# aaletov/open-pcc-metric

Hardware: AMD Instinct MI355X
Metric: Mpoints/s for symmetric D1+D2 PSNR, N_ref=N_deg=1M (higher is better)
Workload: dtype f64

## Files before the change

open_pcc_metric_amd/csrc/pccm_brick.hip:

```cpp
#include "pccm_brick.h"

namespace pccm {

#define BRICK_STAMP(k)                                                                       \
    do {                                                                                     \
        if (STAMP) {                                                                         \
            const unsigned long long now_ = __builtin_amdgcn_s_memtime();                    \
            t_sum[k] += now_ - t_last;         \
            t_last = now_;                                                                   \
        }                                                                                    \
    } while (0)

__device__ __forceinline__ void load_normal(const NNOut &o, int row, double &a, double &b, double &c)
{
    if (o.nrm32) {
        const float4 t = o.nrm32[row];
        a = (double)t.x; b = (double)t.y; c = (double)t.z;
    } else {
        const double *np = o.nrm + 3 * (int64_t)row;
        a = np[0]; b = np[1]; c = np[2];
    }
}

template <bool SELF, int BY, int BZ, bool STAMP, int ABL, bool N32, int PL>
// ... 299 lines not shown
        }
        BRICK_STAMP(5);
        const float thr = __builtin_fmaf(best, 1.0f + 0x1.0p-18f, 2.0e-36f);
        bool settled = false;
        if (ABL & 4) {
            if (best < 0.0f) store_result(out, qrow, 0.0, 0.0, 0);
            settled = true;
        } else if (bestpos != 0xffffffffu && best < 1.0e30f && second > thr) {
            uint32_t f = (bestpos - 8u - lds0) >> 2;
            float partner;
            {
                const v2f px = *reinterpret_cast<const v2f *>(s_x + f), py = *reinterpret_cast<const v2f *>(s_y + f),
                          pz = *reinterpret_cast<const v2f *>(s_z + f);
                const v2f dx = qxx - px, dy = qyy - py, dz = qzz - pz;
                v2f dd = dx * dx;
                dd = __builtin_elementwise_fma(dy, dy, dd);
                dd = __builtin_elementwise_fma(dz, dz, dd);
                float d0 = dd.x, d1 = dd.y;
                if (SELF) {
                    d0 = (__float_as_int(s_r[f]) == qrow) ? kBigF : d0;
                    d1 = (__float_as_int(s_r[f + 1]) == qrow) ? kBigF : d1;
                }
                const bool first = d0 == best;
                partner = first ? d1 : d0;
                f += first ? 0u : 1u;
            }
            float L = face32(q.x, cx, dimx, bp.h32[0], bp.face_lo[0], bp.face_hi[0]);
            L = fminf(L, face32(q.y, cy, dimy, bp.h32[1], bp.face_lo[1], bp.face_hi[1]));
            L = fminf(L, face32(q.z, cz, dimz, bp.h32[2], bp.face_lo[2], bp.face_hi[2]));
            settled = partner > thr && L > 0.0f && best * 1.00001f < L * L * 0.99999f;
            const float wx = s_x[f], wy = s_y[f], wz = s_z[f];
            const int wrow = __float_as_int(s_r[f]);
            if (settled && defer) {
                store_result_rec(out, qrow, wx, wy, wz, wrow);
            } else if (settled) {
                const double rx = (double)wx, ry = (double)wy, rz = (double)wz;
                const double d64 = gdist64(qx, qy, qz, rx, ry, rz);
                double p = 0.0;
                if (fuse) {
                    double e0 = N32 ? (double)nraw.x : n0, e1 = N32 ? (double)nraw.y : n1, e2 = N32 ? (double)nraw.z : n2;
                    if (!fuse_row) {
                        load_normal(out, wrow, e0, e1, e2);
                    }
                    const double ex = __dsub_rn(qx, rx), ey = __dsub_rn(qy, ry), ez = __dsub_rn(qz, rz);
                    p = __dmul_rn(ex, e0);
                    p = __fma_rn(ey, e1, p);
                    p = __fma_rn(ez, e2, p);
                }
                store_result(out, qrow, d64, p, wrow);
            }
        }
        if (!settled) {
            const uint32_t pos = atomicAdd(&J.counters[1], 1u);
            reinterpret_cast<float4 *>(J.tail)[pos] = q;
        }
        if (hn) {
            rn = query_row(qnext);
            qn = load_query(qnext, rn);
            gather_row_normal(__float_as_int(qn.w), fuse_row);
        }
        qi = qnext;
        have = hn;
        if (STAMP) {
            BRICK_STAMP(q_iter == 0 ? 3 : 4);
            ++q_iter;
        }
    }
// ... 189 lines not shown
```

open_pcc_metric_amd/csrc/pccm_color.hip:

```cpp
#include "pccm_internal.h"

namespace pccm {

__constant__ double kColourMatrix[2][9] = {
    {0.2126, 0.7152, 0.0722, -0.1146, -0.3854, 0.5, 0.5, -0.4542, -0.0458},
    {0.25, 0.5, 0.25, 1, 0, -1, -0.5, 1, -0.5},
};

__device__ __forceinline__ void to_scheme(int scheme, const double c[3], double o[3])
{
    if (scheme == 0) {
        o[0] = c[0]; o[1] = c[1]; o[2] = c[2];
        return;
    }
    const double *m = kColourMatrix[scheme - 1];
#pragma unroll
    for (int r = 0; r < 3; ++r) o[r] = fma(m[3 * r + 2], c[2], fma(m[3 * r], c[0], m[3 * r + 1] * c[1]));
}

__device__ __forceinline__ unsigned long long max_key(double v)
{
    return isnan(v) ? 0x7ff8000000000000ull : (unsigned long long)__double_as_longlong(v);
}

struct ByteLut {
    double v[256];
    constexpr ByteLut() : v() {
        for (int k = 0; k < 256; ++k) v[k] = (double)k / 255.0;
    }
};
__constant__ ByteLut c_byte_lut = ByteLut();

template <bool U8>
__global__ __launch_bounds__(256) void k_color_rows(const double *__restrict__ own, const double *__restrict__ other,
                                                    const uint32_t *__restrict__ own8, const uint32_t *__restrict__ other8,
                                                    const int32_t *__restrict__ rows, const float4 *__restrict__ recs, int64_t n, int64_t n_other,
                                                    int scheme, double scale, int what, double *__restrict__ out,
                                                    unsigned long long *__restrict__ maxkeys, unsigned int *__restrict__ bad,
                                                    const double *__restrict__ other_q)
{
    __shared__ unsigned long long s_max[4][3];
    __shared__ double s_lut[U8 ? 256 : 1];
    if (U8) {
        s_lut[threadIdx.x] = c_byte_lut.v[threadIdx.x];
        __syncthreads();
    }
    const int64_t i = (int64_t)blockIdx.x * 256 + threadIdx.x;
    unsigned long long key[3] = {0ull, 0ull, 0ull};
    if (i < n) {
        double a[3], b[3], ta[3], tb[3];
        int64_t r = rows ? rows[i] : (int64_t)__float_as_int(recs[i].w);
        if (r < 0 || r >= n_other) {
            atomicOr(bad, 1u);
            r = 0;
        }
        if (U8) {
            const uint32_t pa = own8[i];
            a[0] = s_lut[pa & 255u]; a[1] = s_lut[(pa >> 8) & 255u]; a[2] = s_lut[(pa >> 16) & 255u];
        } else {
            a[0] = own[3 * i]; a[1] = own[3 * i + 1]; a[2] = own[3 * i + 2];
        }
        if (other_q) {
            b[0] = other_q[3 * i]; b[1] = other_q[3 * i + 1]; b[2] = other_q[3 * i + 2];
        } else if (U8) {
            const uint32_t pb = other8[r];
            b[0] = s_lut[pb & 255u]; b[1] = s_lut[(pb >> 8) & 255u]; b[2] = s_lut[(pb >> 16) & 255u];
        } else {
            b[0] = other[3 * r]; b[1] = other[3 * r + 1]; b[2] = other[3 * r + 2];
        }
        to_scheme(scheme, a, ta);
        to_scheme(scheme, b, tb);
#pragma unroll
        for (int c = 0; c < 3; ++c) {
            const double diff = scale * (ta[c] - tb[c]);
            const double sq = diff * diff;
            if (what == 4) {
                out[(int64_t)c * n + i] = sq;
                key[c] = max_key(sq);
            } else {
                out[3 * i + c] = what == 0 ? ta[c] : what == 1 ? tb[c] : what == 2 ? diff : sq;
            }
        }
    }
    if (what != 4 || !maxkeys) return;
// ... 623 lines not shown
```

open_pcc_metric_amd/csrc/pccm_grid.h:

```cpp
#pragma once
#include "pccm_internal.h"

namespace pccm {

struct GridGeom {
    int dim[3];
    int morton = 0;
    double org[3], h[3], inv_h[3], slack[3];
};

__device__ __forceinline__ uint32_t spread3(uint32_t v)
{
    v &= 0x3ffu;
    v = (v | (v << 16)) & 0x030000ffu;
    v = (v | (v << 8)) & 0x0300f00fu;
    v = (v | (v << 4)) & 0x030c30c3u;
    v = (v | (v << 2)) & 0x09249249u;
    return v;
}

__device__ __forceinline__ int cell_coord(double v, double org, double inv_h, int dim)
{
    double t = floor(__dmul_rn(__dsub_rn(v, org), inv_h));
    t = t < 0.0 ? 0.0 : t;
// ... 64 lines not shown
    *reinterpret_cast<float4 *>(&recs[p]) = r;
}

struct BuildJob {
    const double *x64;
    const float *x32;
    int64_t row0, n;
    uint32_t *cs;
    uint32_t *occ = nullptr;
    const Rec32 *sp = nullptr;
};

struct BuildJobs {
    BuildJob j[2];
    int njobs;
    int64_t total;
};

int sort_by_cell(pccm_ctx *ctx, const BuildJobs &jobs, const GridGeom &g, int64_t ncells, void *recs, bool rec32,
                 uint32_t *zero = nullptr, int nzero = 0);

int64_t scan_tiles(int64_t m);

struct NNOut {
    double *rec;
    int stride;
    const double *nrm;
    const float4 *nrm32;
    int64_t row_base;
    int normal_mode;
    int layout;
};

__device__ __forceinline__ void store_result_rec(const NNOut &o, int qrow, float rx, float ry, float rz, int wrow)
{
    reinterpret_cast<float4 *>(o.rec)[qrow - o.row_base] = make_float4(rx, ry, rz, __int_as_float(wrow));
}

__device__ __forceinline__ void store_result(const NNOut &o, int qrow, double d2, double p, int wrow)
{
    double *dst = o.rec + (int64_t)(qrow - o.row_base) * o.stride;
    *reinterpret_cast<double2 *>(dst) = make_double2(d2, p);
    if (o.stride == 4) *reinterpret_cast<double2 *>(dst + 2) = make_double2(__longlong_as_double((long long)(uint32_t)wrow), 0.0);
}

__device__ __forceinline__ void emit_result(const NNOut &o, int qrow, double qx, double qy, double qz, int wrow, double d2,
                                            double rx, double ry, double rz)
{
    if (o.layout == 1) {
        const bool has = wrow >= 0;
        store_result_rec(o, qrow, (float)(has ? rx : qx), (float)(has ? ry : qy), (float)(has ? rz : qz), wrow);
        return;
    }
    double p = 0.0;
    if (o.nrm && wrow >= 0) {
        const int64_t k = (o.normal_mode == PCCM_NORMAL_ROW) ? (int64_t)qrow : (int64_t)wrow;
        const double ex = __dsub_rn(qx, rx), ey = __dsub_rn(qy, ry), ez = __dsub_rn(qz, rz);
        p = __dmul_rn(ex, o.nrm[3 * k]);
        p = __fma_rn(ey, o.nrm[3 * k + 1], p);
        p = __fma_rn(ez, o.nrm[3 * k + 2], p);
    }
    store_result(o, qrow, d2, p, wrow);
}


__device__ __forceinline__ void emit_result_lookup(const NNOut &o, const double *__restrict__ s64, int qrow, double qx, double qy,
                                                   double qz, int wrow, double d2)
{
    double rx = 0.0, ry = 0.0, rz = 0.0;
    if ((o.nrm || o.layout == 1) && wrow >= 0) {
        rx = s64[3 * (int64_t)wrow];
        ry = s64[3 * (int64_t)wrow + 1];
        rz = s64[3 * (int64_t)wrow + 2];
    }
    emit_result(o, qrow, qx, qy, qz, wrow, d2, rx, ry, rz);
}

struct QueryJob {
    const void *qrecs;
    const void *qbase;
    const uint32_t *qcs;
    int64_t nq, nchunks;
    const uint32_t *cs;
    const uint32_t *occ;
// ... 68 lines not shown
```

open_pcc_metric_amd/csrc/pccm_internal.h:

```cpp
#pragma once
#include <hip/hip_runtime.h>
#include <stdint.h>
#include <mutex>
#include <string>
#include <vector>

#include "pccm.h"
#include "pccm_slot.h"

#ifdef PCCM_DIAG
#define PCCM_DIAG_ENV(name) getenv(name)
#else
#define PCCM_DIAG_ENV(name) (static_cast<const char *>(nullptr))
#endif

namespace pccm {

constexpr int kScanThreads = 256;
constexpr int kScanTile = 1024;
constexpr int kTileVec = kScanTile / 4 * 3;
constexpr int kGranule = 64;
constexpr float kBig32 = 3.0e38f;
constexpr float kPadCoord = 1.0e18f;
constexpr double kMaxAbsCoord = 1.0e15;


struct Cloud {
    int64_t n = 0;
    int64_t n_pad = 0;
    float4 *xyz32 = nullptr;
    double *xyz64 = nullptr;
    float4 *xyz32r = nullptr;
    size_t cap32r = 0;
    double *nrm64 = nullptr;
    float4 *nrm32 = nullptr;
    bool nrm_exact32 = false;
    int64_t n_nrm = 0;
    const void *nrm_host = nullptr;
    int nrm_host_dtype = 0;
    bool nrm_deferred = false;
// ... 570 lines not shown
```

open_pcc_metric_amd/csrc/pccm_point.hip:

```cpp
#include "pccm_internal.h"
#include "pccm_reduce_shape.h"

namespace pccm {

__device__ __forceinline__ unsigned long long order_key(double v)
{
    unsigned long long b = (unsigned long long)__double_as_longlong(v);
    return (b >> 63) ? ~b : (b | 0x8000000000000000ull);
}

template <typename T>
__global__ __launch_bounds__(256) void k_ingest_points(const T *__restrict__ src, int64_t n, int64_t n_pad,
                                                       float *__restrict__ x32, double *__restrict__ x64, float4 *__restrict__ x32r,
                                                       unsigned long long *__restrict__ stats)
{
    __shared__ unsigned long long s_mx[4], s_lo[4][3], s_hi[4][3];
    __shared__ int s_cnt[4][3];
    unsigned long long mx = 0;
    unsigned long long lo[3] = {~0ull, ~0ull, ~0ull}, hi[3] = {0ull, 0ull, 0ull};
    int inexact = 0, bad = 0, frac = 0;
    for (int64_t i = (int64_t)blockIdx.x * 256 + threadIdx.x; i < n_pad; i += (int64_t)gridDim.x * 256) {
        if (i < n) {
            double v[3];
            float f[3];
#pragma unroll
            for (int a = 0; a < 3; ++a) {
                v[a] = (double)src[3 * i + a];
                f[a] = (float)v[a];
                inexact += ((double)f[a] != v[a]) ? 1 : 0;
                frac += (floor(v[a]) != v[a]) ? 1 : 0;
                bad += isfinite(v[a]) ? 0 : 1;
                unsigned long long b = (unsigned long long)__double_as_longlong(fabs(v[a]));
                mx = b > mx ? b : mx;
                x64[3 * i + a] = v[a];
// ... 73 lines not shown
}

int launch_ingest_points(pccm_ctx *ctx, const void *src, int dtype, int64_t n, int64_t n_pad, float4 *x32,
                         double *x64, float4 *x32r, unsigned long long *stats)
{
    ProfScope ps(ctx, PCCM_K_INGEST);
    const int64_t blocks = (n_pad + 255) / 256;
    dim3 grid((unsigned)(blocks < 256 ? blocks : 256));
    if (dtype == PCCM_F32)
        PCCM_LAUNCH(ctx, (k_ingest_points<float>), grid, dim3(256), 0, ctx->stream, (const float *)src, n, n_pad, (float *)x32, x64, x32r, stats);
    else
        PCCM_LAUNCH(ctx, (k_ingest_points<double>), grid, dim3(256), 0, ctx->stream, (const double *)src, n, n_pad, (float *)x32, x64, x32r, stats);
    PCCM_HIP(hipGetLastError());
    return PCCM_OK;
}

int launch_ingest_normals(pccm_ctx *ctx, const void *src, int dtype, int64_t n, double *out, float *out32, unsigned long long *stats)
{
    ProfScope ps(ctx, PCCM_K_INGEST);
    const int64_t n3 = 3 * n;
    dim3 grid((unsigned)((n3 + 255) / 256));
    if (dtype == PCCM_F32)
        PCCM_LAUNCH(ctx, (k_ingest_normals<float>), grid, dim3(256), 0, ctx->stream, (const float *)src, n3, out, out32, stats);
    else
        PCCM_LAUNCH(ctx, (k_ingest_normals<double>), grid, dim3(256), 0, ctx->stream, (const double *)src, n3, out, out32, stats);
    PCCM_HIP(hipGetLastError());
    return PCCM_OK;
}

__device__ __forceinline__ void point_row(const PointJob &J, int64_t i)
{
    const int64_t gi = J.q_begin + i;
    if (J.metric == PCCM_METRIC_ANGULAR) {
        const int64_t j = J.recs ? (int64_t)__float_as_int(J.recs[i].w) : (int64_t)J.idx[i];
        J.val[i] = angular_similarity(J.inrm + 3 * gi, J.nrm + 3 * j);
        return;
    }
    if (is_ssim_metric(J.metric)) {
        const int64_t j = J.recs ? (int64_t)__float_as_int(J.recs[i].w) : (int64_t)J.idx[i];
        J.val[i] = ssim_similarity(J.inrm[gi], J.nrm[j]);
        return;
    }
    const int64_t j = J.idx[i];
    const double *r = J.c64 ? J.c64 + 3 * i : J.r64 + 3 * j;
    const double ex = __dsub_rn(J.q64[3 * gi], r[0]);
    const double ey = __dsub_rn(J.q64[3 * gi + 1], r[1]);
    const double ez = __dsub_rn(J.q64[3 * gi + 2], r[2]);
    if (J.metric == PCCM_METRIC_D1) {
        J.val[3 * i] = ex;
        J.val[3 * i + 1] = ey;
        J.val[3 * i + 2] = ez;
        return;
    }
    const double *nv = (J.normal_mode == PCCM_NORMAL_ROW) ? J.nrm + 3 * gi : J.cn64 ? J.cn64 + 3 * i : J.nrm + 3 * j;
    double p = __dmul_rn(ex, nv[0]);
    p = __fma_rn(ey, nv[1], p);
    p = __fma_rn(ez, nv[2], p);
    J.val[i] = (J.metric == PCCM_METRIC_PROJ) ? p : __dmul_rn(p, p);
}

__global__ __launch_bounds__(256) void k_point_jobs(PointJobs jobs)
{
    const int64_t i0 = (int64_t)blockIdx.x * 256 + threadIdx.x;
    if (i0 >= jobs.off[jobs.njobs]) return;
    int jb = 0;
#pragma unroll
    for (int k = 1; k < 4; ++k)
        if (k < jobs.njobs && i0 >= jobs.off[k]) jb = k;
    point_row(jobs.j[jb], i0 - jobs.off[jb]);
}

int launch_point_jobs(pccm_ctx *ctx, const PointJobs &jobs)
{
    const int64_t total = jobs.off[jobs.njobs];
    if (total <= 0) return PCCM_OK;
    ProfScope ps(ctx, PCCM_K_POINT);
    PCCM_LAUNCH(ctx, k_point_jobs, dim3((unsigned)((total + 255) / 256)), dim3(256), 0, ctx->stream, jobs);
    PCCM_HIP(hipGetLastError());
    return PCCM_OK;
}

struct UnitView {
    const double *val;
    int stride, off0, off1, sq0, sq1;
    int defer;
    int64_t nrm_rows;
    const double *nrm64;
    const float4 *nrm32;
    const float4 *q32;
    int64_t row0;
};

__device__ __forceinline__ void matched_fields(const float4 rec, const float4 *__restrict__ q32, int defer, const double *__restrict__ nrm64,
                                               const float4 *__restrict__ nrm32, int64_t row, bool want_proj, double &d2, double &proj,
                                               int64_t nrm_rows = 0)
{
    const float4 q = q32[row];
    const double qx = (double)q.x, qy = (double)q.y, qz = (double)q.z;
    const double ex = __dsub_rn(qx, (double)rec.x), ey = __dsub_rn(qy, (double)rec.y), ez = __dsub_rn(qz, (double)rec.z);
    d2 = __dadd_rn(__dadd_rn(__dmul_rn(ex, ex), __dmul_rn(ey, ey)), __dmul_rn(ez, ez));
    proj = 0.0;
    if (want_proj && defer != 3) {
        double n0, n1, n2;
        int64_t nr = row;
        if (defer >= 4) {
            nr = (int64_t)__float_as_int(rec.w);
            nr = nr < 0 ? 0 : (nr >= nrm_rows ? nrm_rows - 1 : nr);
        }
        if (defer == 1 || defer == 4) {
            const float4 t = nrm32[nr];
            n0 = (double)t.x; n1 = (double)t.y; n2 = (double)t.z;
        } else {
            n0 = nrm64[3 * nr]; n1 = nrm64[3 * nr + 1]; n2 = nrm64[3 * nr + 2];
        }
        proj = __dmul_rn(ex, n0);
        proj = __fma_rn(ey, n1, proj);
        proj = __fma_rn(ez, n2, proj);
    }
}

__device__ __forceinline__ UnitView unit_view(const UnitJob &J)
{
    UnitView w;
    w.val = J.val;
    w.stride = J.stride;
    w.off0 = J.c[0].off; w.off1 = J.c[1].off;
    w.sq0 = J.c[0].square; w.sq1 = J.c[1].square;
    w.defer = J.defer; w.nrm64 = J.nrm64; w.nrm32 = J.nrm32; w.q32 = J.q32; w.row0 = J.row0; w.nrm_rows = J.nrm_rows;
    return w;
}

__device__ __forceinline__ void unit_load(const UnitView &J, int64_t i, double v[2])
{
    if (J.stride >= 2 && J.defer) {
        matched_fields(reinterpret_cast<const float4 *>(J.val)[i], J.q32, J.defer, J.nrm64, J.nrm32, J.row0 + i, true, v[0], v[1], J.nrm_rows);
    } else if (J.stride >= 2) {
        const double2 t = *reinterpret_cast<const double2 *>(&J.val[i * J.stride]);
        v[0] = t.x;
        v[1] = t.y;
    } else {
        v[0] = v[1] = J.val[i];
    }
}

__device__ __forceinline__ void unit_pick(const UnitView &J, double v[2])
{
    if (J.stride >= 2) {
        const double x = v[0], y = v[1];
        v[0] = J.off0 ? y : x;
        v[1] = J.off1 ? y : x;
// ... 133 lines not shown
#pragma unroll
    for (int r = 0; r < kSelPerCol; ++r) {
        if (!own[r]) continue;
        uint32_t *g = S.hist + ((size_t)p * kSelMax + s0 + r) * kSelBins;
        for (int b = t; b < kSelBins; b += 256) {
            const uint32_t c = lh[r * kSelBins + b];
            if (c) atomicAdd(&g[b], c);
        }
    }
}

__device__ __forceinline__ double dmin_raw(double a, double b)
{
    double r;
    asm("v_min_f64 %0, %1, %2" : "=v"(r) : "v"(a), "v"(b));
    return r;
}
__device__ __forceinline__ double dmax_raw(double a, double b)
{
    double r;
    asm("v_max_f64 %0, %1, %2" : "=v"(r) : "v"(a), "v"(b));
    return r;
}

struct UnitCols {
    static constexpr int NC = 2;
    const UnitView V;
    const int ncols;
    __device__ __forceinline__ explicit UnitCols(const UnitJob &J) : V(unit_view(J)), ncols(J.ncols) {}
    __device__ __forceinline__ bool live(int c) const { return c < ncols; }
    static __device__ __forceinline__ double min(double a, double b) { return fmin(a, b); }
    static __device__ __forceinline__ double max(double a, double b) { return fmax(a, b); }
    __device__ __forceinline__ void one(int64_t i, double v[2]) const { unit_load(V, i, v); unit_pick(V, v); }
    __device__ __forceinline__ void leaf(int64_t base, int k, double v[kLeaf / 8][2]) const
    {
        __builtin_assume((base & (kLeaf - 1)) == 0 && k >= 0 && k < 8);
        if (V.stride >= 2 && V.defer) {
#pragma unroll
            for (int j = 0; j < kLeaf / 8; ++j) unit_load(V, base + 8 * j + k, v[j]);
        } else if (V.stride >= 2) {
#pragma unroll
            for (int j = 0; j < kLeaf / 8; ++j) {
                const double2 t = *reinterpret_cast<const double2 *>(&V.val[(base + 8 * j + k) * V.stride]);
                v[j][0] = t.x;
                v[j][1] = t.y;
            }
        } else {
#pragma unroll
            for (int j = 0; j < kLeaf / 8; ++j) v[j][0] = v[j][1] = V.val[base + 8 * j + k];
        }
#pragma unroll
        for (int j = 0; j < kLeaf / 8; ++j) unit_pick(V, v[j]);
    }
};

template <int STRIDE, int CFG, int DEFER>
struct LeanCols {
    static constexpr int NC = CFG == 0 ? 2 : 1;
    const double *__restrict__ val, *__restrict__ nrm64;
    const float4 *__restrict__ nrm32, *__restrict__ q32;
    const int64_t row0, nrm_rows;
    __device__ __forceinline__ explicit LeanCols(const UnitJob &J)
        : val(J.val), nrm64(J.nrm64), nrm32(J.nrm32), q32(J.q32), row0(J.row0), nrm_rows(J.nrm_rows) {}
    __device__ __forceinline__ bool live(int) const { return true; }
    static __device__ __forceinline__ double min(double a, double b) { return dmin_raw(a, b); }
    static __device__ __forceinline__ double max(double a, double b) { return dmax_raw(a, b); }
    __device__ __forceinline__ void one(int64_t i, double out[NC]) const { at(val + i * STRIDE, i, out); }
    __device__ __forceinline__ void at(const double *p, int64_t i, double out[NC]) const
    {
        double x, y = 0.0;
        if (DEFER) {
            matched_fields(*reinterpret_cast<const float4 *>(p), q32, DEFER, nrm64, nrm32, row0 + i, CFG != 1, x, y, nrm_rows);
        } else if (STRIDE >= 2) {
            const double2 q = *reinterpret_cast<const double2 *>(p);
            x = q.x; y = q.y;
        } else {
            x = *p;
        }
        if (CFG == 0) { out[0] = x; out[1] = __dmul_rn(y, y); }
        else out[0] = CFG == 1 ? x : __dmul_rn(y, y);
    }
    __device__ __forceinline__ void leaf(int64_t base, int k, double v[kLeaf / 8][NC]) const
    {
        __builtin_assume((base & (kLeaf - 1)) == 0 && k >= 0 && k < 8);
        const int64_t first = base + k;
        const double *p = val + first * STRIDE;
#pragma unroll
        for (int j = 0; j < kLeaf / 8; ++j) at(p + (int64_t)j * 8 * STRIDE, first + 8 * j, v[j]);
    }
};

__device__ __forceinline__ int unit_job_at(const int64_t (&off)[9], int njobs, int64_t pos)
{
    int jb = 0;
#pragma unroll
    for (int k = 1; k < 8; ++k)
        if (k < njobs && pos >= off[k]) jb = k;
    return jb;
}

template <class P>
__device__ __forceinline__ void unit_leaves(const UnitJobs &jobs, int jb, int64_t t)
{
    constexpr int NC = P::NC;
    __shared__ double ls[NC][32], lmn[NC][32], lmx[NC][32];
    const UnitJob &J = jobs.j[jb];
    const P cols(J);
    const int64_t ns = J.ns, nunits = J.nunits;
    const int64_t lane = t - jobs.uoff[jb], u = lane >> 3;
    const int k = threadIdx.x & 7, grp = threadIdx.x >> 3;
    const int64_t base = u * kLeaf;
    const bool live = u < nunits;
    const int64_t cnt = !live ? 0 : ((ns - base < kLeaf) ? ns - base : kLeaf);
    double r[NC], mn[NC], mx[NC];
    if (cnt == kLeaf) {
        double v[kLeaf / 8][NC];
        cols.leaf(base, k, v);
#pragma unroll
        for (int c = 0; c < NC; ++c) {
            r[c] = v[0][c];
            mn[c] = mx[c] = v[0][c];
#pragma unroll
            for (int j = 1; j < kLeaf / 8; ++j) {
                r[c] = __dadd_rn(r[c], v[j][c]);
                mn[c] = P::min(mn[c], v[j][c]);
                mx[c] = P::max(mx[c], v[j][c]);
            }
        }
    } else {
#pragma unroll
        for (int c = 0; c < NC; ++c) { r[c] = 0.0; mn[c] = INFINITY; mx[c] = -INFINITY; }
        for (int64_t e = k; e < cnt; e += 8) {
            double w[NC];
            cols.one(base + e, w);
#pragma unroll
            for (int c = 0; c < NC; ++c) {
                r[c] = __dadd_rn(r[c], w[c]);
                mn[c] = P::min(mn[c], w[c]);
                mx[c] = P::max(mx[c], w[c]);
            }
        }
    }
#pragma unroll
    for (int c = 0; c < NC; ++c) {
#pragma unroll
        for (int off = 1; off < 8; off <<= 1) {
            r[c] = __dadd_rn(r[c], __shfl_xor(r[c], off));
            mn[c] = P::min(mn[c], __shfl_xor(mn[c], off));
            mx[c] = P::max(mx[c], __shfl_xor(mx[c], off));
        }
    }
    if (k == 0) {
#pragma unroll
        for (int c = 0; c < NC; ++c) {
            double *ou = cols.live(c) ? J.c[c].out_units : nullptr;
            if (live && ou) {
                ou[u] = r[c];
                ou[nunits + u] = mn[c];
                ou[2 * nunits + u] = mx[c];
            }
            ls[c][grp] = r[c];
// ... 21 lines not shown
    }
}

template <class P>
__device__ __forceinline__ void unit_tail(const UnitJobs &jobs, int64_t c0)
{
    if (c0 >= jobs.toff[jobs.njobs]) return;
    const int jb = unit_job_at(jobs.toff, jobs.njobs, c0);
    const UnitJob &J = jobs.j[jb];
    const P cols(J);
    const int64_t e = c0 - jobs.toff[jb];
    double v[P::NC];
    cols.one(J.tail_first + e, v);
#pragma unroll
    for (int c = 0; c < P::NC; ++c)
        if (cols.live(c)) J.c[c].out_tail[e] = v[c];
}

__global__ __launch_bounds__(256) void k_unit_jobs(UnitJobs jobs)
{
    __shared__ __attribute__((aligned(16))) unsigned char sel_smem[kSelLds];
    if (jobs.sel.pass) {
        unit_select(jobs, sel_smem);
        return;
    }
    const int64_t t = (int64_t)blockIdx.x * 256 + threadIdx.x;
    const int64_t unit_threads = jobs.uoff[jobs.njobs];
    if (t < unit_threads)
        unit_leaves<UnitCols>(jobs, __builtin_amdgcn_readfirstlane(unit_job_at(jobs.uoff, jobs.njobs, t)), t);
    else
        unit_tail<UnitCols>(jobs, t - unit_threads);
}

template <int STRIDE, int CFG, int DEFER = 0>
__global__ __launch_bounds__(256) void k_unit_lean(UnitJobs jobs)
{
    const int64_t t = (int64_t)blockIdx.x * 256 + threadIdx.x;
    const int64_t unit_threads = jobs.uoff[jobs.njobs];
    if ((int64_t)blockIdx.x * 256 < unit_threads)
        unit_leaves<LeanCols<STRIDE, CFG, DEFER>>(jobs, unit_job_at(jobs.uoff, jobs.njobs, (int64_t)blockIdx.x * 256), t);
    else
        unit_tail<LeanCols<STRIDE, CFG, DEFER>>(jobs, t - unit_threads);
}

__global__ __launch_bounds__(64) void k_publish(unsigned long long *done)
{
    if (threadIdx.x == 0) {
        __builtin_amdgcn_fence(__ATOMIC_RELEASE, "");
        asm volatile("s_waitcnt vmcnt(0)" ::: "memory");
        __hip_atomic_fetch_add(done, 1ull, __ATOMIC_RELAXED, __HIP_MEMORY_SCOPE_SYSTEM);
    }
}

struct LeanKernel {
    ReduceShape shape;
    void (*stub)(UnitJobs);
};
template <int STRIDE, int CFG, int DEFER>
constexpr LeanKernel lean() { return {{STRIDE, CFG, DEFER}, k_unit_lean<STRIDE, CFG, DEFER>}; }
static constexpr LeanKernel kLeanKernels[] = {
    lean<1, 1, 0>(),
    lean<2, 0, 0>(),
    lean<2, 1, 0>(),
    lean<2, 2, 0>(),
    lean<4, 0, 0>(),
    lean<4, 1, 0>(),
    lean<4, 2, 0>(),
    lean<2, 0, 1>(),
// ... 79 lines not shown
int launch_unit_select(pccm_ctx *ctx, UnitJobs &jobs)
{
    UnitSelect &S = jobs.sel;
    if (S.nsel <= 0) return PCCM_OK;
    ProfScope ps(ctx, PCCM_K_REDUCE);
    int nb = 0;
    for (int k = 0; k < 8; ++k) {
        S.boff[k] = nb;
        if (k < jobs.njobs) {
            const int64_t want = (jobs.j[k].ns + 4095) / 4096;
            nb += (int)(want < 1 ? 1 : want > 256 ? 256 : want);
        }
    }
    S.boff[8] = nb;
    PCCM_HIP(hipMemsetAsync(S.hist, 0, (size_t)kSelPasses * kSelMax * kSelBins * sizeof(uint32_t), ctx->stream));
    for (int p = 0; p <= kSelPasses; ++p) {
        S.pass = p + 1;
        PCCM_LAUNCH(ctx, k_unit_jobs, dim3(p < kSelPasses ? (unsigned)nb : 1u), dim3(256), 0, ctx->stream, jobs);
    }
    S.pass = 0;
    PCCM_HIP(hipGetLastError());
    return PCCM_OK;
}

__global__ __launch_bounds__(256) void k_unpack(const double *__restrict__ rec, int stride, int layout, const float4 *__restrict__ q32, int64_t row0,
                                                int64_t ns, int32_t *__restrict__ idx, double *__restrict__ d2)
{
    const int64_t i = (int64_t)blockIdx.x * 256 + threadIdx.x;
    if (i >= ns) return;
    if (layout == 1) {
        const float4 r = reinterpret_cast<const float4 *>(rec)[i];
        double x, y;
        matched_fields(r, q32, 3, nullptr, nullptr, row0 + i, false, x, y);
        if (idx) idx[i] = __float_as_int(r.w);
        d2[i] = x;
        return;
    }
    const double *r = rec + i * stride;
    if (stride == 4 && idx) idx[i] = (int32_t)(__double_as_longlong(r[2]) & 0xffffffffll);
    d2[i] = r[0];
}

int launch_unpack(pccm_ctx *ctx, const double *rec, int stride, int layout, const float4 *q32, int64_t row0, int64_t ns, int32_t *idx, double *d2)
{
    if (ns <= 0) return PCCM_OK;
    PCCM_LAUNCH(ctx, k_unpack, dim3((unsigned)((ns + 255) / 256)), dim3(256), 0, ctx->stream, rec, stride, layout, q32, row0, ns, idx, d2);
    PCCM_HIP(hipGetLastError());
    return PCCM_OK;
}

}
```

open_pcc_metric_amd/csrc/pccm_rescan.h:

```cpp
#pragma once
#include "pccm_internal.h"

namespace pccm {

__device__ __forceinline__ float dist32(float qx, float qy, float qz, float rx, float ry, float rz)
{
    float dx = qx - rx, dy = qy - ry, dz = qz - rz;
    float d = dx * dx;
    d = __builtin_fmaf(dy, dy, d);
    d = __builtin_fmaf(dz, dz, d);
    return d;
}

__device__ __forceinline__ void load_pt32(const float *__restrict__ p, int64_t j, float &x, float &y, float &z)
{
    const float *qd = p + (j >> 2) * 12 + (j & 3);
    x = qd[0];
    y = qd[4];
    z = qd[8];
}

__device__ __forceinline__ double dist64(double qx, double qy, double qz, double rx, double ry, double rz)
{
    double dx = __dsub_rn(qx, rx), dy = __dsub_rn(qy, ry), dz = __dsub_rn(qz, rz);
// ... 34 lines not shown
        if (SELF) cand = cand && (j != J.q_begin + i);
        if (cand) {
            const double e = dist64(qx, qy, qz, J.r64[3 * j], J.r64[3 * j + 1], J.r64[3 * j + 2]);
            if (e < bd) { bd = e; bj = (int)j; }
        }
    }
}

__device__ __forceinline__ void block_lexmin(double &bd, int &bj, double *s_d, int *s_j)
{
    const int tid = threadIdx.x, lane = tid & 63, w = tid >> 6;
    const double m = wave_min_f64(bd);
    const int cj = wave_min_i32(bd == m ? bj : 0x7fffffff);
    __syncthreads();
    if (lane == 0) { s_d[w] = m; s_j[w] = cj; }
    __syncthreads();
    if (tid == 0) {
        bd = s_d[0];
        bj = s_j[0];
        for (int k = 1; k < 4; ++k)
            if (s_d[k] < bd || (s_d[k] == bd && s_j[k] < bj)) { bd = s_d[k]; bj = s_j[k]; }
    }
}

__device__ __forceinline__ void rescan_emit(const RescanJob &J, int64_t i, int bj, double bd)
{
    if (!J.rec_out) {
        J.idx_out[i] = bj;
        J.d2_out[i] = bd;
        return;
    }
    if (J.rec_layout == 1) {
        const bool has = bj >= 0 && bj != 0x7fffffff;
        const double *src = has ? J.r64 + 3 * (int64_t)bj : J.q64 + 3 * (J.q_begin + i);
        reinterpret_cast<float4 *>(J.rec_out)[i] = make_float4((float)src[0], (float)src[1], (float)src[2], __int_as_float(has ? bj : -1));
        return;
    }
    double p = 0.0;
    if (J.nrm && bj >= 0 && bj != 0x7fffffff) {
        const int64_t gi = J.q_begin + i, k = (J.normal_mode == PCCM_NORMAL_ROW) ? gi : (int64_t)bj;
        const double ex = __dsub_rn(J.q64[3 * gi], J.r64[3 * (int64_t)bj]);
        const double ey = __dsub_rn(J.q64[3 * gi + 1], J.r64[3 * (int64_t)bj + 1]);
        const double ez = __dsub_rn(J.q64[3 * gi + 2], J.r64[3 * (int64_t)bj + 2]);
        p = __dmul_rn(ex, J.nrm[3 * k]);
        p = __fma_rn(ey, J.nrm[3 * k + 1], p);
        p = __fma_rn(ez, J.nrm[3 * k + 2], p);
    }
    double *dst = J.rec_out + i * J.rec_stride;
    *reinterpret_cast<double2 *>(dst) = make_double2(bd, p);
    if (J.rec_stride == 4) *reinterpret_cast<double2 *>(dst + 2) = make_double2(__longlong_as_double((long long)(uint32_t)bj), 0.0);
}

template <bool SELF>
__device__ __forceinline__ void rescan_body(const RescanJob &J, uint32_t b, uint32_t nb)
{
    __shared__ double s_d[4];
    __shared__ int s_j[4];
    __shared__ uint32_t s_ticket;
    const uint32_t count = __hip_atomic_load(J.nflag, __ATOMIC_RELAXED, __HIP_MEMORY_SCOPE_AGENT);
    if (count == 0) return;
    const int tid = threadIdx.x;
    if (count > (uint32_t)kSplitMax) {
        for (uint32_t f = b; f < count; f += nb) {
            const int64_t i = __hip_atomic_load(&J.flagged[f], __ATOMIC_RELAXED, __HIP_MEMORY_SCOPE_AGENT);
            double bd;
            int bj;
            rescan_slice<SELF>(J, i, __hip_atomic_load(&J.flag_thr[f], __ATOMIC_RELAXED, __HIP_MEMORY_SCOPE_AGENT), 0, J.nr, tid, bd, bj);
            block_lexmin(bd, bj, s_d, s_j);
// ... 38 lines not shown
```

open_pcc_metric_amd/csrc/pccm_vox.hip:

```cpp
#include "pccm_grid.h"

namespace pccm {

constexpr int kVoxRowsPadded = 200;
__constant__ __attribute__((aligned(16))) uint32_t c_vox_rows[kVoxRowsPadded] = {
    0x808, 0x10708, 0x10807, 0x10809, 0x10908, 0x20707, 0x20709, 0x20907, 0x20909, 0x40608, 0x40806, 0x4080a, 0x40a08, 0x50607, 0x50609,
    0x50706, 0x5070a, 0x50906, 0x5090a, 0x50a07, 0x50a09, 0x80606, 0x8060a, 0x80a06, 0x80a0a, 0x90508, 0x90805, 0x9080b, 0x90b08, 0xa0507,
    0xa0509, 0xa0705, 0xa070b, 0xa0905, 0xa090b, 0xa0b07, 0xa0b09, 0xd0506, 0xd050a, 0xd0605, 0xd060b, 0xd0a05, 0xd0a0b, 0xd0b06, 0xd0b0a,
    0x100408, 0x100804, 0x10080c, 0x100c08, 0x110407, 0x110409, 0x110704, 0x11070c, 0x110904, 0x11090c, 0x110c07, 0x110c09, 0x120505, 0x12050b,
    0x120b05, 0x120b0b, 0x140406, 0x14040a, 0x140604, 0x14060c, 0x140a04, 0x140a0c, 0x140c06, 0x140c0a, 0x190308, 0x190803, 0x19080d, 0x190d08,
    0x190405, 0x19040b, 0x190504, 0x19050c, 0x190b04, 0x190b0c, 0x190c05, 0x190c0b, 0x1a0307, 0x1a0309, 0x1a0703, 0x1a070d, 0x1a0903, 0x1a090d,
    0x1a0d07, 0x1a0d09, 0x1d0306, 0x1d030a, 0x1d0603, 0x1d060d, 0x1d0a03, 0x1d0a0d, 0x1d0d06, 0x1d0d0a, 0x200404, 0x20040c, 0x200c04, 0x200c0c,
    0x220305, 0x22030b, 0x220503, 0x22050d, 0x220b03, 0x220b0d, 0x220d05, 0x220d0b, 0x240208, 0x240802, 0x24080e, 0x240e08, 0x250207, 0x250209,
    0x250702, 0x25070e, 0x250902, 0x25090e, 0x250e07, 0x250e09, 0x280206, 0x28020a, 0x280602, 0x28060e, 0x280a02, 0x280a0e, 0x280e06, 0x280e0a,
    0x290304, 0x29030c, 0x290403, 0x29040d, 0x290c03, 0x290c0d, 0x290d04, 0x290d0c, 0x2d0205, 0x2d020b, 0x2d0502, 0x2d050e, 0x2d0b02, 0x2d0b0e,
    0x2d0e05, 0x2d0e0b, 0x310108, 0x310801, 0x31080f, 0x310f08, 0x320107, 0x320109, 0x320701, 0x32070f, 0x320901, 0x32090f, 0x320f07, 0x320f09,
    0x320303, 0x32030d, 0x320d03, 0x320d0d, 0x340204, 0x34020c, 0x340402, 0x34040e, 0x340c02, 0x340c0e, 0x340e04, 0x340e0c, 0x350106, 0x35010a,
    0x350601, 0x35060f, 0x350a01, 0x350a0f, 0x350f06, 0x350f0a, 0x3a0105, 0x3a010b, 0x3a0501, 0x3a050f, 0x3a0b01, 0x3a0b0f, 0x3a0f05, 0x3a0f0b,
    0x3d0203, 0x3d020d, 0x3d0302, 0x3d030e, 0x3d0d02, 0x3d0d0e, 0x3d0e03, 0x3d0e0d, 0x400008, 0x400800, 0x400810, 0x401008,
    0xffff0808, 0xffff0808, 0xffff0808
};

constexpr int kVoxNear = 16, kVoxNearEntries = 153;
__constant__ uint16_t c_vox_near[kVoxNearEntries] = {
// ... 300 lines not shown
                    }
                }
                int wrow = 0x7fffffff;
                uint32_t wv3 = 0u;
                const uint32_t usable = cnt <= (uint32_t)kVoxTies ? cnt : 0u;
                for (int j0 = 0; j0 < kVoxTies; j0 += 4) {
                    if (__ballot((uint32_t)j0 < usable) == 0ull) break;
                    int rows_of[4];
                    uint32_t vox_of[4];
#pragma unroll
                    for (int jj = 0; jj < 4; ++jj) {
                        const int j = j0 + jj;
                        rows_of[jj] = 0x7fffffff;
                        vox_of[jj] = 0u;
                        if ((uint32_t)j < usable) {
                            const uint32_t h = s_hit[j * 64 + lane];
                            const int dz = (int)(h & 0x1fu) - 8, dy = (int)((h >> 5) & 0x1fu) - 8, dxs = (int)((h >> 10) & 0xfu);
                            const int X = (h & 0x8000u) ? lx - dxs : lx + dxs, Y = ly + dy, Z = lz + dz;
                            const int rr = (Y >> 3) + 3 * (Z >> 3), bb = rr * 3 + (X >> 3), v = (X & 7) + 8 * (Y & 7) + 64 * (Z & 7);
                            const uint32_t rank = (uint32_t)s_pre[bb * 16 + (v >> 5)] + (uint32_t)__popc(s_brick[bb * 16 + (v >> 5)] & ((1u << (v & 31)) - 1u));
                            rows_of[jj] = J.vminrow[s_cs[rr * 4 + (X >> 3)] + rank];
                            vox_of[jj] = (uint32_t)X | ((uint32_t)Y << 5) | ((uint32_t)Z << 10);
                        }
                    }
#pragma unroll
                    for (int jj = 0; jj < 4; ++jj)
                        if (rows_of[jj] < wrow) {
                            wrow = rows_of[jj];
                            wv3 = vox_of[jj];
                        }
                }
                if (have) {
                    if (ok && cnt >= 1u && cnt <= (uint32_t)kVoxTies && wrow != 0x7fffffff) {
                        store_result_rec(J.out, __float_as_int(q.w), (float)(rx0 + (int)(wv3 & 31u)), (float)(ry0 + (int)((wv3 >> 5) & 31u)),
                                         (float)(rz0 + (int)(wv3 >> 10)), wrow);
                    } else {
                        if (ok && (cnt == 0u || (cnt <= (uint32_t)kVoxTies && wrow == 0x7fffffff)) && jobs.err) atomicOr(jobs.err, kErrVoxState);
                        const uint32_t pos = atomicAdd(&J.counters[1], 1u);
                        reinterpret_cast<float4 *>(J.tail)[pos] = q;
                    }
                }
            } else if (have) {
                const uint32_t d2 = best >> 8;
                const int qrow = __float_as_int(q.w);
                if (d2 <= 64u) {
                    const uint32_t e = c_vox_rows[best & 0xffu];
                    const int dy = (int)((e >> 8) & 0xffu) - 8, dz = (int)(e & 0xffu) - 8;
                    uint32_t w = s_rows[base + dz * 24 + dy];
                    if (SELF && (best & 0xffu) == 0u) w &= own;
                    const int up = __builtin_ctz(w >> L), dn = __builtin_clz(w & below) + L - 31;
                    const int mx = dn < up ? lx - dn : lx + up;
                    store_result_rec(J.out, qrow, (float)(rx0 + mx), (float)(ry0 + ly + dy), (float)(rz0 + lz + dz), -1);
                } else {
                    const uint32_t pos = atomicAdd(&J.counters[1], 1u);
                    reinterpret_cast<float4 *>(J.tail)[pos] = q;
                }
            }
        }
        __syncthreads();
    }
}

int launch_vox_bricks(pccm_ctx *ctx, const VoxBuild &vb, const GridGeom &g)
{
    dim3 grid((unsigned)((vb.ncells + kVoxTile - 1) / kVoxTile), (unsigned)vb.njobs);
    PCCM_LAUNCH(ctx, k_vox_bricks, grid, dim3(256), 0, ctx->stream, vb, g);
    PCCM_LAUNCH(ctx, k_vox_list, dim3(kVoxListWGs, (unsigned)vb.njobs), dim3(1024), 0, ctx->stream, vb);
    PCCM_HIP(hipGetLastError());
    return PCCM_OK;
}

int launch_vox_query(pccm_ctx *ctx, const QueryJobs &jobs, const GridGeom &g, bool self, bool rows)
{
    dim3 grid(8192u, (unsigned)jobs.njobs);
    if (self && rows) return fail(PCCM_E_STATE, "the self search with matched rows does not run on voxel bricks");
    if (self) PCCM_LAUNCH(ctx, (k_vox_query<true, false>), grid, dim3(64), 0, ctx->stream, jobs, g);
    else if (rows) PCCM_LAUNCH(ctx, (k_vox_query<false, true>), grid, dim3(64), 0, ctx->stream, jobs, g);
    else PCCM_LAUNCH(ctx, (k_vox_query<false, false>), grid, dim3(64), 0, ctx->stream, jobs, g);
    PCCM_HIP(hipGetLastError());
    return PCCM_OK;
}

}
```

Before: 10960.

## Store exact float error vectors in NN result records to skip query reloads

Nearest-neighbour result records now hold the query-minus-reference error vector in float form when the float subtraction is exact, flagged through an encoded row word. The reduction leaf can then compute d2 and projection without re-reading the query coordinates, and uses a batched loader that falls back to the matched form only when a wave contains such records. It also sets waves-per-EU occupancy hints on the lean unit kernel. The cost is extra arithmetic at store time and in row decoding, plus a more complex record format that every consumer must decode correctly.

```diff
diff --git a/open_pcc_metric_amd/csrc/pccm_brick.hip b/open_pcc_metric_amd/csrc/pccm_brick.hip
--- a/open_pcc_metric_amd/csrc/pccm_brick.hip
+++ b/open_pcc_metric_amd/csrc/pccm_brick.hip
@@ -355,7 +355,7 @@
             const float wx = s_x[f], wy = s_y[f], wz = s_z[f];
             const int wrow = __float_as_int(s_r[f]);
             if (settled && defer) {
-                store_result_rec(out, qrow, wx, wy, wz, wrow);
+                store_result_rec(out, qrow, errrec_encode(q.x, q.y, q.z, wx, wy, wz, wrow));
             } else if (settled) {
                 const double rx = (double)wx, ry = (double)wy, rz = (double)wz;
                 const double d64 = gdist64(qx, qy, qz, rx, ry, rz);
diff --git a/open_pcc_metric_amd/csrc/pccm_color.hip b/open_pcc_metric_amd/csrc/pccm_color.hip
--- a/open_pcc_metric_amd/csrc/pccm_color.hip
+++ b/open_pcc_metric_amd/csrc/pccm_color.hip
@@ -49,7 +49,7 @@
     unsigned long long key[3] = {0ull, 0ull, 0ull};
     if (i < n) {
         double a[3], b[3], ta[3], tb[3];
-        int64_t r = rows ? rows[i] : (int64_t)__float_as_int(recs[i].w);
+        int64_t r = rows ? rows[i] : (int64_t)errrec_row(recs[i]);
         if (r < 0 || r >= n_other) {
             atomicOr(bad, 1u);
             r = 0;
diff --git a/open_pcc_metric_amd/csrc/pccm_errrec.h b/open_pcc_metric_amd/csrc/pccm_errrec.h
--- /dev/null
+++ b/open_pcc_metric_amd/csrc/pccm_errrec.h
@@ -0,0 +1,106 @@
+#pragma once
+#include <hip/hip_runtime.h>
+#include <stdint.h>
+#include <string.h>
+
+namespace pccm {
+
+constexpr int32_t kErrNoRow = INT32_MIN;
+constexpr int32_t kErrMaxRow = INT32_MAX - 2;
+
+__host__ __device__ __forceinline__ uint32_t errrec_bits(float v)
+{
+#if defined(__HIP_DEVICE_COMPILE__)
+    return __float_as_uint(v);
+#else
+    uint32_t u;
+    memcpy(&u, &v, sizeof u);
+    return u;
+#endif
+}
+
+__host__ __device__ __forceinline__ float errrec_sub(float q, float r, float &err)
+{
+    const float e = q - r;
+    const float bb = e - q;
+    err = (q - (e - bb)) - (r + bb);
+    return e;
+}
+
+__host__ __device__ __forceinline__ bool errrec_exact(float qx, float qy, float qz, float rx, float ry, float rz, float &ex, float &ey, float &ez)
+{
+    float dx, dy, dz;
+    ex = errrec_sub(qx, rx, dx);
+    ey = errrec_sub(qy, ry, dy);
+    ez = errrec_sub(qz, rz, dz);
+    return ((errrec_bits(dx) | errrec_bits(dy) | errrec_bits(dz)) << 1) == 0u;
+}
+
+__host__ __device__ __forceinline__ float errrec_word_float(int32_t w)
+{
+    float f;
+    memcpy(&f, &w, sizeof f);
+    return f;
+}
+
+__host__ __device__ __forceinline__ int32_t errrec_row_word(int32_t row) { return row < 0 ? kErrNoRow : -2 - row; }
+
+__host__ __device__ __forceinline__ float4 errrec_encode(float qx, float qy, float qz, float rx, float ry, float rz, int32_t row)
+{
+    float ex, ey, ez;
+    const bool err_form = errrec_exact(qx, qy, qz, rx, ry, rz, ex, ey, ez) && row <= kErrMaxRow;
+    const int32_t w = err_form ? errrec_row_word(row) : (row < 0 ? -1 : row);
+    float4 rec;
+    rec.x = err_form ? ex : rx;
+    rec.y = err_form ? ey : ry;
+    rec.z = err_form ? ez : rz;
+    rec.w = errrec_word_float(w);
+    return rec;
+}
+
+__host__ __device__ __forceinline__ float4 errrec_encode_exact(float qx, float qy, float qz, float rx, float ry, float rz, int32_t row)
+{
+    const bool err_form = row <= kErrMaxRow;
+    const int32_t w = err_form ? errrec_row_word(row) : row;
+    float4 rec;
+    rec.x = err_form ? qx - rx : rx;
+    rec.y = err_form ? qy - ry : ry;
+    rec.z = err_form ? qz - rz : rz;
+    rec.w = errrec_word_float(w);
+    return rec;
+}
+
+__host__ __device__ __forceinline__ int32_t errrec_word(const float4 &rec)
+{
+    const float f = rec.w;
+    int32_t w;
+    memcpy(&w, &f, sizeof w);
+    return w;
+}
+
+__host__ __device__ __forceinline__ bool errrec_is_error_form(int32_t w) { return w <= -2; }
+
+__host__ __device__ __forceinline__ int32_t errrec_row(int32_t w) { return w >= -1 ? w : (w == kErrNoRow ? -1 : -2 - w); }
+__host__ __device__ __forceinline__ int32_t errrec_row(const float4 &rec) { return errrec_row(errrec_word(rec)); }
+
+__host__ __device__ __forceinline__ void errrec_error_form(const float4 &rec, double &ex, double &ey, double &ez)
+{
+    ex = (double)rec.x; ey = (double)rec.y; ez = (double)rec.z;
+}
+
+__host__ __device__ __forceinline__ void errrec_matched_form(const float4 &rec, float qx, float qy, float qz, double &ex, double &ey, double &ez)
+{
+    ex = (double)qx - (double)rec.x; ey = (double)qy - (double)rec.y; ez = (double)qz - (double)rec.z;
+}
+
+__host__ __device__ __forceinline__ void errrec_error(const float4 &rec, const float4 *__restrict__ q32, int64_t row, double &ex, double &ey, double &ez)
+{
+    if (errrec_is_error_form(errrec_word(rec))) {
+        errrec_error_form(rec, ex, ey, ez);
+    } else {
+        const float4 q = q32[row];
+        errrec_matched_form(rec, q.x, q.y, q.z, ex, ey, ez);
+    }
+}
+
+}
diff --git a/open_pcc_metric_amd/csrc/pccm_grid.h b/open_pcc_metric_amd/csrc/pccm_grid.h
--- a/open_pcc_metric_amd/csrc/pccm_grid.h
+++ b/open_pcc_metric_amd/csrc/pccm_grid.h
@@ -120,9 +120,9 @@
     int layout;
 };
 
-__device__ __forceinline__ void store_result_rec(const NNOut &o, int qrow, float rx, float ry, float rz, int wrow)
-{
-    reinterpret_cast<float4 *>(o.rec)[qrow - o.row_base] = make_float4(rx, ry, rz, __int_as_float(wrow));
+__device__ __forceinline__ void store_result_rec(const NNOut &o, int qrow, const float4 rec)
+{
+    reinterpret_cast<float4 *>(o.rec)[qrow - o.row_base] = rec;
 }
 
 __device__ __forceinline__ void store_result(const NNOut &o, int qrow, double d2, double p, int wrow)
@@ -137,7 +137,8 @@
 {
     if (o.layout == 1) {
         const bool has = wrow >= 0;
-        store_result_rec(o, qrow, (float)(has ? rx : qx), (float)(has ? ry : qy), (float)(has ? rz : qz), wrow);
+        store_result_rec(o, qrow, errrec_encode((float)qx, (float)qy, (float)qz, (float)(has ? rx : qx), (float)(has ? ry : qy),
+                                                (float)(has ? rz : qz), has ? wrow : -1));
         return;
     }
     double p = 0.0;
diff --git a/open_pcc_metric_amd/csrc/pccm_internal.h b/open_pcc_metric_amd/csrc/pccm_internal.h
--- a/open_pcc_metric_amd/csrc/pccm_internal.h
+++ b/open_pcc_metric_amd/csrc/pccm_internal.h
@@ -6,6 +6,7 @@
 #include <vector>
 
 #include "pccm.h"
+#include "pccm_errrec.h"
 #include "pccm_slot.h"
 
 #ifdef PCCM_DIAG
diff --git a/open_pcc_metric_amd/csrc/pccm_point.hip b/open_pcc_metric_amd/csrc/pccm_point.hip
--- a/open_pcc_metric_amd/csrc/pccm_point.hip
+++ b/open_pcc_metric_amd/csrc/pccm_point.hip
@@ -1,5 +1,7 @@
 #include "pccm_internal.h"
 #include "pccm_reduce_shape.h"
+
+#include <type_traits>
 
 namespace pccm {
 
@@ -139,12 +141,12 @@
 {
     const int64_t gi = J.q_begin + i;
     if (J.metric == PCCM_METRIC_ANGULAR) {
-        const int64_t j = J.recs ? (int64_t)__float_as_int(J.recs[i].w) : (int64_t)J.idx[i];
+        const int64_t j = J.recs ? (int64_t)errrec_row(J.recs[i]) : (int64_t)J.idx[i];
         J.val[i] = angular_similarity(J.inrm + 3 * gi, J.nrm + 3 * j);
         return;
     }
     if (is_ssim_metric(J.metric)) {
-        const int64_t j = J.recs ? (int64_t)__float_as_int(J.recs[i].w) : (int64_t)J.idx[i];
+        const int64_t j = J.recs ? (int64_t)errrec_row(J.recs[i]) : (int64_t)J.idx[i];
         J.val[i] = ssim_similarity(J.inrm[gi], J.nrm[j]);
         return;
     }
@@ -198,31 +200,108 @@
     int64_t row0;
 };
 
+__device__ __forceinline__ double error_d2(double ex, double ey, double ez)
+{
+    return __dadd_rn(__dadd_rn(__dmul_rn(ex, ex), __dmul_rn(ey, ey)), __dmul_rn(ez, ez));
+}
+
+__device__ __forceinline__ double error_proj(double ex, double ey, double ez, double n0, double n1, double n2)
+{
+    double p = __dmul_rn(ex, n0);
+    p = __fma_rn(ey, n1, p);
+    return __fma_rn(ez, n2, p);
+}
+
+__device__ __forceinline__ int64_t normal_row(const float4 rec, int defer, int64_t row, int64_t nrm_rows)
+{
+    if (defer < 4) return row;
+    const int64_t nr = (int64_t)errrec_row(rec);
+    return nr < 0 ? 0 : (nr >= nrm_rows ? nrm_rows - 1 : nr);
+}
+
+template <class NT>
+struct NormalOf {
+    NT x, y, z;
+};
+template <class NT>
+__device__ __forceinline__ NormalOf<NT> load_normal_of(int defer, const double *__restrict__ nrm64, const float4 *__restrict__ nrm32, int64_t nr)
+{
+    NormalOf<NT> n;
+    if (defer == 1 || defer == 4) {
+        const float4 t = nrm32[nr];
+        n.x = (NT)t.x; n.y = (NT)t.y; n.z = (NT)t.z;
+    } else {
+        n.x = (NT)nrm64[3 * nr]; n.y = (NT)nrm64[3 * nr + 1]; n.z = (NT)nrm64[3 * nr + 2];
+    }
+    return n;
+}
+
 __device__ __forceinline__ void matched_fields(const float4 rec, const float4 *__restrict__ q32, int defer, const double *__restrict__ nrm64,
                                                const float4 *__restrict__ nrm32, int64_t row, bool want_proj, double &d2, double &proj,
                                                int64_t nrm_rows = 0)
 {
-    const float4 q = q32[row];
-    const double qx = (double)q.x, qy = (double)q.y, qz = (double)q.z;
-    const double ex = __dsub_rn(qx, (double)rec.x), ey = __dsub_rn(qy, (double)rec.y), ez = __dsub_rn(qz, (double)rec.z);
-    d2 = __dadd_rn(__dadd_rn(__dmul_rn(ex, ex), __dmul_rn(ey, ey)), __dmul_rn(ez, ez));
+    double ex, ey, ez;
+    errrec_error(rec, q32, row, ex, ey, ez);
+    d2 = error_d2(ex, ey, ez);
     proj = 0.0;
     if (want_proj && defer != 3) {
-        double n0, n1, n2;
-        int64_t nr = row;
-        if (defer >= 4) {
-            nr = (int64_t)__float_as_int(rec.w);
-            nr = nr < 0 ? 0 : (nr >= nrm_rows ? nrm_rows - 1 : nr);
-        }
-        if (defer == 1 || defer == 4) {
-            const float4 t = nrm32[nr];
-            n0 = (double)t.x; n1 = (double)t.y; n2 = (double)t.z;
+        const NormalOf<double> n = load_normal_of<double>(defer, nrm64, nrm32, normal_row(rec, defer, row, nrm_rows));
+        proj = error_proj(ex, ey, ez, n.x, n.y, n.z);
+    }
+}
+
+constexpr int kLeafBatch = 2;
+template <class NT, int G, bool PRELOAD, class Emit>
+__device__ __forceinline__ void matched_leaf(const float4 *__restrict__ recs, const float4 *__restrict__ q32, int defer,
+                                             const double *__restrict__ nrm64, const float4 *__restrict__ nrm32, int64_t first, bool want_proj,
+                                             int64_t nrm_rows, Emit emit)
+{
+    constexpr int N = kLeaf / 8;
+    static_assert(N % G == 0 && G % 2 == 0, "whole batches of pairs");
+    const bool projects = want_proj && defer != 3, streams = PRELOAD && projects && defer < 4;
+#pragma unroll
+    for (int j0 = 0; j0 < N; j0 += G) {
+        float4 rec[G];
+        NormalOf<NT> nv[G];
+        double ex[G], ey[G], ez[G];
+#pragma unroll
+        for (int u = 0; u < G; ++u) rec[u] = recs[(j0 + u) * 8];
+        if (streams) {
+#pragma unroll
+            for (int u = 0; u < G; ++u) nv[u] = load_normal_of<NT>(defer, nrm64, nrm32, first + 8 * (j0 + u));
+        }
+        bool matched_form = false;
+#pragma unroll
+        for (int u = 0; u < G; ++u) matched_form = matched_form || !errrec_is_error_form(errrec_word(rec[u]));
+        if (__builtin_expect(__ballot(matched_form) != 0ull, 0)) {
+#pragma unroll
+            for (int u0 = 0; u0 < G; u0 += 2) {
+                float4 q[2];
+#pragma unroll
+                for (int v = 0; v < 2; ++v) q[v] = q32[first + 8 * (j0 + u0 + v)];
+#pragma unroll
+                for (int v = 0; v < 2; ++v) {
+                    const int u = u0 + v;
+                    double mx, my, mz;
+                    errrec_error_form(rec[u], ex[u], ey[u], ez[u]);
+                    errrec_matched_form(rec[u], q[v].x, q[v].y, q[v].z, mx, my, mz);
+                    const bool ef = errrec_is_error_form(errrec_word(rec[u]));
+                    ex[u] = ef ? ex[u] : mx; ey[u] = ef ? ey[u] : my; ez[u] = ef ? ez[u] : mz;
+                }
+            }
         } else {
-            n0 = nrm64[3 * nr]; n1 = nrm64[3 * nr + 1]; n2 = nrm64[3 * nr + 2];
-        }
-        proj = __dmul_rn(ex, n0);
-        proj = __fma_rn(ey, n1, proj);
-        proj = __fma_rn(ez, n2, proj);
+#pragma unroll
+            for (int u = 0; u < G; ++u) errrec_error_form(rec[u], ex[u], ey[u], ez[u]);
+        }
+#pragma unroll
+        for (int u = 0; u < G; ++u) {
+            double p = 0.0;
+            if (projects) {
+                const NormalOf<NT> n = streams ? nv[u] : load_normal_of<NT>(defer, nrm64, nrm32, normal_row(rec[u], defer, first + 8 * (j0 + u), nrm_rows));
+                p = error_proj(ex[u], ey[u], ez[u], (double)n.x, (double)n.y, (double)n.z);
+            }
+            emit(j0 + u, error_d2(ex[u], ey[u], ez[u]), p);
+        }
     }
 }
 
@@ -422,13 +501,21 @@
     static __device__ __forceinline__ double min(double a, double b) { return fmin(a, b); }
     static __device__ __forceinline__ double max(double a, double b) { return fmax(a, b); }
     __device__ __forceinline__ void one(int64_t i, double v[2]) const { unit_load(V, i, v); unit_pick(V, v); }
-    __device__ __forceinline__ void leaf(int64_t base, int k, double v[kLeaf / 8][2]) const
+    template <class F>
+    __device__ __forceinline__ void leaf(int64_t base, int k, F fold) const
     {
         __builtin_assume((base & (kLeaf - 1)) == 0 && k >= 0 && k < 8);
         if (V.stride >= 2 && V.defer) {
-#pragma unroll
-            for (int j = 0; j < kLeaf / 8; ++j) unit_load(V, base + 8 * j + k, v[j]);
-        } else if (V.stride >= 2) {
+            matched_leaf<double, kLeafBatch, true>(reinterpret_cast<const float4 *>(V.val) + base + k, V.q32, V.defer, V.nrm64, V.nrm32, V.row0 + base + k, true,
+                                 V.nrm_rows, [&](int j, double d2, double proj) {
+                                     double w[2] = {d2, proj};
+                                     unit_pick(V, w);
+                                     fold(j, w);
+                                 });
+            return;
+        }
+        double v[kLeaf / 8][2];
+        if (V.stride >= 2) {
 #pragma unroll
             for (int j = 0; j < kLeaf / 8; ++j) {
                 const double2 t = *reinterpret_cast<const double2 *>(&V.val[(base + 8 * j + k) * V.stride]);
@@ -440,7 +527,10 @@
             for (int j = 0; j < kLeaf / 8; ++j) v[j][0] = v[j][1] = V.val[base + 8 * j + k];
         }
 #pragma unroll
-        for (int j = 0; j < kLeaf / 8; ++j) unit_pick(V, v[j]);
+        for (int j = 0; j < kLeaf / 8; ++j) {
+            unit_pick(V, v[j]);
+            fold(j, v[j]);
+        }
     }
 };
 
@@ -456,6 +546,11 @@
     static __device__ __forceinline__ double min(double a, double b) { return dmin_raw(a, b); }
     static __device__ __forceinline__ double max(double a, double b) { return dmax_raw(a, b); }
     __device__ __forceinline__ void one(int64_t i, double out[NC]) const { at(val + i * STRIDE, i, out); }
+    static __device__ __forceinline__ void pick(double x, double y, double out[NC])
+    {
+        if (CFG == 0) { out[0] = x; out[1] = __dmul_rn(y, y); }
+        else out[0] = CFG == 1 ? x : __dmul_rn(y, y);
+    }
     __device__ __forceinline__ void at(const double *p, int64_t i, double out[NC]) const
     {
         double x, y = 0.0;
@@ -467,16 +562,31 @@
         } else {
             x = *p;
         }
-        if (CFG == 0) { out[0] = x; out[1] = __dmul_rn(y, y); }
-        else out[0] = CFG == 1 ? x : __dmul_rn(y, y);
-    }
-    __device__ __forceinline__ void leaf(int64_t base, int k, double v[kLeaf / 8][NC]) const
+        pick(x, y, out);
+    }
+    template <class F>
+    __device__ __forceinline__ void leaf(int64_t base, int k, F fold) const
     {
         __builtin_assume((base & (kLeaf - 1)) == 0 && k >= 0 && k < 8);
         const int64_t first = base + k;
         const double *p = val + first * STRIDE;
-#pragma unroll
-        for (int j = 0; j < kLeaf / 8; ++j) at(p + (int64_t)j * 8 * STRIDE, first + 8 * j, v[j]);
+        if constexpr (DEFER != 0) {
+            static_assert(STRIDE == 2, "a result record of layout 1 is 16 bytes");
+            using NT = typename std::conditional<DEFER == 1 || DEFER == 4, float, double>::type;
+            constexpr bool kNormalsFirst = !(CFG == 2 && DEFER == 1);
+            matched_leaf<NT, kLeafBatch, kNormalsFirst>(reinterpret_cast<const float4 *>(p), q32, DEFER, nrm64, nrm32, row0 + first, CFG != 1, nrm_rows,
+                             [&](int j, double d2, double proj) {
+                                 double w[NC];
+                                 pick(d2, proj, w);
+                                 fold(j, w);
+                             });
+        } else {
+            double v[kLeaf / 8][NC];
+#pragma unroll
+            for (int j = 0; j < kLeaf / 8; ++j) at(p + (int64_t)j * 8 * STRIDE, first + 8 * j, v[j]);
+#pragma unroll
+            for (int j = 0; j < kLeaf / 8; ++j) fold(j, v[j]);
+        }
     }
 };
 
@@ -504,19 +614,14 @@
     const int64_t cnt = !live ? 0 : ((ns - base < kLeaf) ? ns - base : kLeaf);
     double r[NC], mn[NC], mx[NC];
     if (cnt == kLeaf) {
-        double v[kLeaf / 8][NC];
-        cols.leaf(base, k, v);
-#pragma unroll
-        for (int c = 0; c < NC; ++c) {
-            r[c] = v[0][c];
-            mn[c] = mx[c] = v[0][c];
-#pragma unroll
-            for (int j = 1; j < kLeaf / 8; ++j) {
-                r[c] = __dadd_rn(r[c], v[j][c]);
-                mn[c] = P::min(mn[c], v[j][c]);
-                mx[c] = P::max(mx[c], v[j][c]);
-            }
-        }
+        cols.leaf(base, k, [&](int j, const double (&v)[NC]) {
+#pragma unroll
+            for (int c = 0; c < NC; ++c) {
+                r[c] = j == 0 ? v[c] : __dadd_rn(r[c], v[c]);
+                mn[c] = j == 0 ? v[c] : P::min(mn[c], v[c]);
+                mx[c] = j == 0 ? v[c] : P::max(mx[c], v[c]);
+            }
+        });
     } else {
 #pragma unroll
         for (int c = 0; c < NC; ++c) { r[c] = 0.0; mn[c] = INFINITY; mx[c] = -INFINITY; }
@@ -604,8 +709,13 @@
         unit_tail<UnitCols>(jobs, t - unit_threads);
 }
 
+constexpr int lean_waves(int cfg, int defer)
+{
+    return defer == 0 ? 8 : cfg == 1 || (cfg == 2 && defer == 1) ? 6 : cfg == 2 && defer == 4 ? 7 : 4;
+}
+
 template <int STRIDE, int CFG, int DEFER = 0>
-__global__ __launch_bounds__(256) void k_unit_lean(UnitJobs jobs)
+__global__ __launch_bounds__(256) __attribute__((amdgpu_waves_per_eu(lean_waves(CFG, DEFER)))) void k_unit_lean(UnitJobs jobs)
 {
     const int64_t t = (int64_t)blockIdx.x * 256 + threadIdx.x;
     const int64_t unit_threads = jobs.uoff[jobs.njobs];
@@ -751,7 +861,7 @@
         const float4 r = reinterpret_cast<const float4 *>(rec)[i];
         double x, y;
         matched_fields(r, q32, 3, nullptr, nullptr, row0 + i, false, x, y);
-        if (idx) idx[i] = __float_as_int(r.w);
+        if (idx) idx[i] = errrec_row(r);
         d2[i] = x;
         return;
     }
diff --git a/open_pcc_metric_amd/csrc/pccm_rescan.h b/open_pcc_metric_amd/csrc/pccm_rescan.h
--- a/open_pcc_metric_amd/csrc/pccm_rescan.h
+++ b/open_pcc_metric_amd/csrc/pccm_rescan.h
@@ -90,8 +90,9 @@
     }
     if (J.rec_layout == 1) {
         const bool has = bj >= 0 && bj != 0x7fffffff;
-        const double *src = has ? J.r64 + 3 * (int64_t)bj : J.q64 + 3 * (J.q_begin + i);
-        reinterpret_cast<float4 *>(J.rec_out)[i] = make_float4((float)src[0], (float)src[1], (float)src[2], __int_as_float(has ? bj : -1));
+        const double *q = J.q64 + 3 * (J.q_begin + i), *src = has ? J.r64 + 3 * (int64_t)bj : q;
+        reinterpret_cast<float4 *>(J.rec_out)[i] =
+            errrec_encode((float)q[0], (float)q[1], (float)q[2], (float)src[0], (float)src[1], (float)src[2], has ? bj : -1);
         return;
     }
     double p = 0.0;
diff --git a/open_pcc_metric_amd/csrc/pccm_vox.hip b/open_pcc_metric_amd/csrc/pccm_vox.hip
--- a/open_pcc_metric_amd/csrc/pccm_vox.hip
+++ b/open_pcc_metric_amd/csrc/pccm_vox.hip
@@ -356,8 +356,9 @@
                 }
                 if (have) {
                     if (ok && cnt >= 1u && cnt <= (uint32_t)kVoxTies && wrow != 0x7fffffff) {
-                        store_result_rec(J.out, __float_as_int(q.w), (float)(rx0 + (int)(wv3 & 31u)), (float)(ry0 + (int)((wv3 >> 5) & 31u)),
-                                         (float)(rz0 + (int)(wv3 >> 10)), wrow);
+                        store_result_rec(J.out, __float_as_int(q.w),
+                                         errrec_encode_exact(q.x, q.y, q.z, (float)(rx0 + (int)(wv3 & 31u)), (float)(ry0 + (int)((wv3 >> 5) & 31u)),
+                                                             (float)(rz0 + (int)(wv3 >> 10)), wrow));
                     } else {
                         if (ok && (cnt == 0u || (cnt <= (uint32_t)kVoxTies && wrow == 0x7fffffff)) && jobs.err) atomicOr(jobs.err, kErrVoxState);
                         const uint32_t pos = atomicAdd(&J.counters[1], 1u);
@@ -374,7 +375,8 @@
                     if (SELF && (best & 0xffu) == 0u) w &= own;
                     const int up = __builtin_ctz(w >> L), dn = __builtin_clz(w & below) + L - 31;
                     const int mx = dn < up ? lx - dn : lx + up;
-                    store_result_rec(J.out, qrow, (float)(rx0 + mx), (float)(ry0 + ly + dy), (float)(rz0 + lz + dz), -1);
+                    store_result_rec(J.out, qrow,
+                                     errrec_encode_exact(q.x, q.y, q.z, (float)(rx0 + mx), (float)(ry0 + ly + dy), (float)(rz0 + lz + dz), -1));
                 } else {
                     const uint32_t pos = atomicAdd(&J.counters[1], 1u);
                     reinterpret_cast<float4 *>(J.tail)[pos] = q;
```

New measurement: 11060, median of 4. About the same (+0.9%).
